# JzHuai0108/sim3opt

Hardware: AMD Instinct MI355X
Metric: LM iterations/s (higher is better)
Workload: dtype f64

## Files before the change

sim3opt_amd/csrc/amg_kernels.hpp:

```cpp
#pragma once

__global__ __launch_bounds__(WG) void k_amg_adjoint(int nb, const int32_t* __restrict__ row2v,
                                                    const Sim3* __restrict__ states,
                                                    double* __restrict__ P) {
  for (int i = blockIdx.x * WG + threadIdx.x; i < nb; i += gridDim.x * WG) {
  const Sim3 S = load_sim3(states + row2v[i]);
  double R[9];
  sim3::R_from_quat(S.q, R);
  double A[49];
#pragma unroll
  for (int k = 0; k < 49; ++k) A[k] = 0.0;
  const double t0 = S.t[0], t1 = S.t[1], t2 = S.t[2];
#pragma unroll
  for (int c = 0; c < 3; ++c) {
    const double v0 = R[c], v1 = R[3 + c], v2 = R[6 + c];
    A[0 + 7 * c] = v0;
    A[1 + 7 * c] = v1;
    A[2 + 7 * c] = v2;
    A[3 + 7 * c] = t1 * v2 - t2 * v1;
    A[4 + 7 * c] = t2 * v0 - t0 * v2;
    A[5 + 7 * c] = t0 * v1 - t1 * v0;
    A[3 + 7 * (3 + c)] = S.s * v0;
    A[4 + 7 * (3 + c)] = S.s * v1;
    A[5 + 7 * (3 + c)] = S.s * v2;
// ... 214 lines not shown
  const int sub = lane / 7, rr = lane % 7, base = lane - rr;
  for (int row0 = row_lo + (blockIdx.x * 4 + wave) * 9; row0 < row_hi; row0 += gridDim.x * 36) {
    const bool act = lane < 63 && row0 + sub < row_hi;
    const int row = act ? (list ? list[row0 + sub] : row0 + sub) : 0;
    const double xc = act ? x_c[(size_t)7 * agg[row] + rr] : 0.0;
    double add = xc;
    if (HASP) {
      add = 0.0;
#pragma unroll
      for (int m = 0; m < 7; ++m) {
        const double xm = __shfl(xc, base + m);
        if (act) add += P[(size_t)49 * row + rr + 7 * m] * xm;
      }
    }
    if (act) x_out[(size_t)7 * row + rr] = x_in[(size_t)7 * row + rr] + scale * add;
  }
}

constexpr int AMG_DENSE_MAX_N = 7 * AMG_MAX_COARSEST;
__global__ __launch_bounds__(WG) void k_amg_dense_fill(int nb, const int32_t* __restrict__ rowptr,
                                                       const int32_t* __restrict__ colidx,
                                                       const double* __restrict__ vals,
                                                       double* __restrict__ A,
                                                       const double* __restrict__ diag64 = nullptr) {
  const int n = 7 * nb;
  const int nnz = 49 * rowptr[nb];
  for (int t = blockIdx.x * WG + threadIdx.x; t < nnz; t += gridDim.x * WG) {
    const int k = t / 49, e = t % 49;
    int lo = 0, hi = nb;
    while (hi - lo > 1) {
      const int mid = (lo + hi) >> 1;
      if (rowptr[mid] <= k) lo = mid; else hi = mid;
    }
    const double v = diag64 && k == rowptr[lo] ? diag64[(size_t)49 * lo + e] : vals[(size_t)49 * k + e];
    A[(size_t)(7 * lo + e % 7) * n + 7 * colidx[k] + e / 7] = v;
  }
}


template <int NP>
__device__ inline bool gj_invert_rows(double (&prow)[NP], int lane) {
  bool spd = true;
#pragma unroll
  for (int k = 0; k < NP; ++k) {
    double pk[NP];
#pragma unroll
    for (int c = 0; c < NP; ++c) pk[c] = __shfl(prow[c], k);
// ... 47 lines not shown
#pragma unroll
    for (int c = 0; c < H; ++c) prow[c] = src[(size_t)rr * ld + H * h + c];
    spd = gj_invert_halfrows<NP>(prow, lane);
    if (r < NP) {
#pragma unroll
      for (int c = 0; c < H; ++c) Pout[r * NP + H * h + c] = prow[c];
    }
  } else {
    double prow[NP];
    const int rr = lane < NP ? lane : 0;
#pragma unroll
    for (int c = 0; c < NP; ++c) prow[c] = src[(size_t)rr * ld + c];
    spd = gj_invert_rows<NP>(prow, lane);
    if (lane < NP) {
#pragma unroll
      for (int c = 0; c < NP; ++c) Pout[lane * NP + c] = prow[c];
    }
  }
  if (!spd && lane == 0) sc->fail = 1;
}

template <int PB>
__global__ __launch_bounds__(64) void k_amg_dense_gj_first(int n, const double* __restrict__ A,
                                                           double* __restrict__ Pout, DevScalars* sc) {
  gj_invert_block<PB>(A, n, Pout, threadIdx.x, sc);
}

template <int PB>
__global__ __launch_bounds__(WG) __attribute__((amdgpu_waves_per_eu(2))) void k_amg_dense_gj_step(int n, int k0, const double* __restrict__ A,
                                                          double* __restrict__ B,
                                                          const double* __restrict__ Pin,
                                                          double* __restrict__ Pout, int pbn,
                                                          DevScalars* sc) {
  __shared__ double P[PB][PB + 1];
  __shared__ double ak[PB][64];
  __shared__ double rowk[PB][64];
  __shared__ double colk[64][PB + 1];
  const int tid = threadIdx.x;
  const bool ahead = blockIdx.y == 0;
  if (ahead && (blockIdx.x != 0 || pbn == 0)) return;
  const int ext = ahead ? pbn : 64;
  const int i0 = ahead ? k0 + PB : (int)(blockIdx.y - 1) * 64, j0 = ahead ? k0 + PB : (int)blockIdx.x * 64;
  const int ty = tid >> 4, tx = tid & 15;
  double v[4][4];
  if (ahead) {
#pragma unroll
    for (int e = 0; e < 4; ++e) {
      const int t = tid + WG * e;
      v[0][e] = t < ext * ext ? A[(size_t)(i0 + t / ext) * n + j0 + t % ext] : 0.0;
    }
  } else {
#pragma unroll
    for (int a = 0; a < 4; ++a)
#pragma unroll
      for (int b = 0; b < 4; ++b) {
        const int i = i0 + ty + 16 * a, j = j0 + tx + 16 * b;
        v[a][b] = i < n && j < n ? A[(size_t)i * n + j] : 0.0;
// ... 101 lines not shown
```

sim3opt_amd/csrc/batch_kernels.hpp:

```cpp
#pragma once

template <int K>
__global__ __launch_bounds__(WG) void k_final_sum2_k(const double* __restrict__ pa, const double* __restrict__ pb,
                                                     int n, int pstride, DevScalars* __restrict__ sc) {
  __shared__ double sh[4];
#pragma unroll
  for (int s = 0; s < K; ++s) {
    const double a = sum_partials(pa + (size_t)s * pstride, n, sh);
    const double b = sum_partials(pb + (size_t)s * pstride, n, sh);
    if (threadIdx.x == 0) {
      sc[s].tmp_pq = a;
      sc[s].tmp_rz = b;
    }
  }
}

template <int K>
__global__ __launch_bounds__(WG) void k_pcg_init_k(int r0, int r1, const double* __restrict__ b,
                                                   const double* __restrict__ Minv, double* __restrict__ x,
                                                   double* __restrict__ r, double* __restrict__ z,
                                                   double* __restrict__ p, double* __restrict__ sv,
                                                   BatchStrides bs) {
  const int lane = threadIdx.x & 63;
  const int wave = threadIdx.x >> 6;
  const int sub = lane / 7, rr = lane % 7, base = lane - rr;
  for (int row0 = r0 + (blockIdx.x * 4 + wave) * 9; row0 < r1; row0 += gridDim.x * 36) {
    const int row = row0 + sub;
    const bool act = lane < 63 && row < r1;
    const size_t j = (size_t)7 * row + rr;
    const double rv = act ? b[j] : 0.0;
#pragma unroll
    for (int s = 0; s < K; ++s) {
      const size_t o = (size_t)s * bs.vec;
      if (act) {
        x[o + j] = 0.0;
        r[o + j] = rv;
// ... 260 lines not shown
```

sim3opt_amd/csrc/engine_amg.hip:

```cpp
#include "engine_impl.hpp"

namespace sim3opt {

#include "spmv_kernel.hpp"
#include "amg_kernels.hpp"

int Engine::amg_init(const Structure& s, bool automatic, std::string& err) {
  (void)err;
  amg_omega = std::max(0.1, std::min(0.95, opt.amg_omega));
  amg_additive = opt.amg_additive != 0;
  {
    const bool partitioned = part_world() >= 2;
    int last = 0;
    for (int l = 1; l <= AMG_MAX_LEVELS; ++l) {
      const int o = l <= 4 ? opt.amg_cycle[l - 1] : 0;
      if (o >= 1 && o <= 3) last = o;
      amg_visits[l] = last > 0 ? last : (partitioned ? (l <= 1 ? 1 : 2) : (l <= 1 ? 2 : 3));
    }
    amg_visits[0] = 1;
  }
  amg_fp32 = opt.amg_fp32 != 0;
  adaptive_prec = opt.adaptive_prec != 0 && automatic;
  amg_pivot = opt.amg_pivot >= 28 ? 28 : 14;
  for (int l = 0; l <= AMG_MAX_LEVELS; ++l)
// ... 158 lines not shown
  }
  if (amg_fp32)
    for (int l = nl - 1; l < nl; ++l) {
      const size_t cnt = (size_t)49 * (size_t)amg[l].nnzb;
      hipLaunchKernelGGL(k_to_f32, dim3(grid_for((int64_t)(cnt / 4), WG)), dim3(WG), 0, stream, cnt,
                         (const double*)amg[l].vals, amg[l].vals32);
    }
  HIPCHK(hipGetLastError());
  amg_stale = false;
  return SIM3OPT_OK;
}

void Engine::amg_prepare(double lambda) {
  const int nl = (int)amg.size();
  for (int l = 0; l < nl; ++l) {
    const AmgLevel& L = amg[l];
    const int lo = L.lo, hi = L.hi;
    jacobi(lo, hi, L.rowptr, L.vals, lambda, L.Minv, l == 0 && amg_additive ? 1.0 : amg_omega, L.diagH, L.W,
           l > 0 ? L.vals32 : (float*)nullptr);
  }
  dense_inverse(nullptr, d_Ainv, d_sc);
}

void Engine::dense_inverse(const double* diag64, double* Aout, DevScalars* sc) {
  const int nl = (int)amg.size();
  const AmgLevel& Lc = amg[nl - 1];
  const int nd = 7 * Lc.nb;
  auto pivot_rows = [&](int k0) { return nd - k0 >= amg_pivot ? amg_pivot : (nd - k0 >= 14 ? 14 : 7); };
  int nsteps = 0;
  for (int k0 = 0; k0 < nd; k0 += pivot_rows(k0)) ++nsteps;
  double *src = nsteps % 2 ? d_Ainv2 : Aout, *dst = nsteps % 2 ? Aout : d_Ainv2;
  (void)hipMemsetAsync(src, 0, sizeof(double) * (size_t)nd * nd, stream);
  hipLaunchKernelGGL(k_amg_dense_fill, dim3(grid_for(49 * Lc.nnzb, WG)), dim3(WG), 0, stream, Lc.nb,
                     Lc.rowptr, Lc.colidx, Lc.vals, src, diag64);
  double *pin = d_piv, *pout = d_piv + 28 * 28;
  switch (pivot_rows(0)) {
    case 28: hipLaunchKernelGGL((k_amg_dense_gj_first<28>), dim3(1), dim3(64), 0, stream, nd, (const double*)src, pin, sc); break;
    case 14: hipLaunchKernelGGL((k_amg_dense_gj_first<14>), dim3(1), dim3(64), 0, stream, nd, (const double*)src, pin, sc); break;
    default: hipLaunchKernelGGL((k_amg_dense_gj_first<7>), dim3(1), dim3(64), 0, stream, nd, (const double*)src, pin, sc);
  }
  const dim3 gt((nd + 63) / 64, (nd + 63) / 64 + 1);
  for (int k0 = 0; k0 < nd;) {
    const int pb = pivot_rows(k0), pbn = k0 + pb < nd ? pivot_rows(k0 + pb) : 0;
    if (pb == 28)
      hipLaunchKernelGGL((k_amg_dense_gj_step<28>), gt, dim3(WG), 0, stream, nd, k0, (const double*)src,
                         dst, (const double*)pin, pout, pbn, sc);
    else if (pb == 14)
      hipLaunchKernelGGL((k_amg_dense_gj_step<14>), gt, dim3(WG), 0, stream, nd, k0, (const double*)src,
                         dst, (const double*)pin, pout, pbn, sc);
    else
      hipLaunchKernelGGL((k_amg_dense_gj_step<7>), gt, dim3(WG), 0, stream, nd, k0, (const double*)src,
                         dst, (const double*)pin, pout, pbn, sc);
    k0 += pb;
    std::swap(src, dst);
    std::swap(pin, pout);
  }
}

void Engine::spmv_mode(const AmgLevel& L, int mode, int level, const double* v, double* out,
               const double* rvec, const double* xc) {
  double* const rz_part = level == 0 && mode == 2 && !amg_additive ? d_part_b : nullptr;
#define AMG_SPMV(NTV, MODEV)                                                                     \
hipLaunchKernelGGL((k_spmv_span<8, NTV, MODEV>), dim3(L.span_grid), dim3(WG), 0, stream, L.nb,  \
                   L.wrow, L.rowptr, L.colidx, L.vals, v, out, 0.0, rz_part, rvec,              \
                   const_cast<double*>(xc), level == 0 ? d_sc : (DevScalars*)nullptr, L.Minv, 1,   \
                   (const int32_t*)L.agg, amg_over, BatchStrides{0, 0, 0, 0, 0}, (const float*)nullptr)
#define AMG_SPMV32(NTV, MODEV)                                                                    \
hipLaunchKernelGGL((k_spmv_span<(NTV) ? SIM3OPT_F32_CH : SIM3OPT_COARSE_CH, NTV, MODEV, float>), dim3(L.span_grid), dim3(WG), 0, stream,  \
                   L.nb, L.wrow, L.rowptr, L.colidx, (const float*)L.vals32, v, out, 0.0,         \
                   rz_part, rvec, const_cast<double*>(xc),                                        \
                   level == 0 ? d_sc : (DevScalars*)nullptr, L.Minv, 1, (const int32_t*)L.agg, amg_over, BatchStrides{0, 0, 0, 0, 0}, (const float*)nullptr)
  if (amg_fp32) {
    if (level == 0) { if (mode == 1) AMG_SPMV32(true, 1); else AMG_SPMV32(true, 2); }
    else { if (mode == 1) AMG_SPMV32(false, 1); else if (mode == 3) AMG_SPMV32(false, 3); else AMG_SPMV32(false, 2); }
  } else {
// ... 135 lines not shown
```

sim3opt_amd/csrc/engine_batch.hip:

```cpp
#include "engine_impl.hpp"

namespace sim3opt {

#include "spmv_kernel.hpp"
#include "batch_kernels.hpp"

static inline int64_t pad64(int64_t n) { return (n + 63) / 64 * 64; }

#define BATCH_DISPATCH(NS, ...) \
  do {                          \
    if ((NS) == 1) { constexpr int KS = 1; __VA_ARGS__; } \
    else if ((NS) == 2) { constexpr int KS = 2; __VA_ARGS__; } \
    else if ((NS) == 3) { constexpr int KS = 3; __VA_ARGS__; } \
    else { constexpr int KS = 4; __VA_ARGS__; } \
  } while (0)

int Engine::batch_alloc(std::string& err) {
  if (batch_ready) return SIM3OPT_OK;
  const int nl = (int)amg.size();
  auto alloc = [&](double*& p, size_t count) -> int {
    HIPCHK(dev_malloc((void**)&p, sizeof(double) * std::max<size_t>(count, 1)));
    batch_owned.push_back(p);
    HIPCHK(hipMemsetAsync(p, 0, sizeof(double) * std::max<size_t>(count, 1), stream));
    return SIM3OPT_OK;
// ... 8 lines not shown
  blv.assign(nl, BatchLevel());
  for (int l = 0; l < nl; ++l) {
    BatchLevel& B = blv[l];
    const AmgLevel& L = amg[l];
    B.vs = l == 0 ? b_vs : pad64(7 * (int64_t)L.nb);
    B.ms = (int64_t)49 * L.nb;
    int rc = alloc(B.Minv, (size_t)KB * B.ms);
    if (rc) return rc;
    if (l == 0) {
      B.r = b_r; B.x = b_z; B.t = b_az;
    } else {
      if ((rc = alloc(B.r, (size_t)KB * B.vs))) return rc;
      if ((rc = alloc(B.x, (size_t)KB * B.vs))) return rc;
      if ((rc = alloc(B.t, (size_t)KB * B.vs))) return rc;
      HIPCHK(dev_malloc((void**)&B.diag32, sizeof(float) * (size_t)KB * B.ms));
      batch_owned.push_back(B.diag32);
      HIPCHK(hipMemsetAsync(B.diag32, 0, sizeof(float) * (size_t)KB * B.ms, stream));
    }
  }
  const size_t nc = (size_t)7 * amg[nl - 1].nb;
  b_as = (int64_t)(nc * nc);
  int rc = alloc(b_Ainv, (size_t)KB * b_as);
  if (rc) return rc;
  if ((rc = alloc(b_diag64, (size_t)KB * 49 * amg[nl - 1].nb))) return rc;
  if ((rc = alloc(b_part_a, (size_t)KB * SPAN_GRID_MAX))) return rc;
  if ((rc = alloc(b_part_b, (size_t)KB * SPAN_GRID_MAX))) return rc;
  HIPCHK(dev_malloc((void**)&d_bsc, sizeof(DevScalars) * KB));
  batch_owned.push_back(d_bsc);
  HIPCHK(hipMemsetAsync(d_bsc, 0, sizeof(DevScalars) * KB, stream));
  HIPCHK(host_malloc((void**)&h_bsc, sizeof(DevScalars) * KB));
  batch_ready = true;
  return SIM3OPT_OK;
}

void Engine::batch_release() {
  for (void* p : batch_owned)
    if (p) dev_free(p);
  batch_owned.clear();
  if (h_bsc) host_free(h_bsc);
  h_bsc = nullptr;
  d_bsc = nullptr;
  blv.clear();
  batch_ready = false;
}

void Engine::b_spmv_mode(int level, int mode, const double* v, double* out, const double* rvec, const double* xc) {
// ... 72 lines not shown
  return other;
}

int Engine::pcg_batch(const double* lams, int nsys, int32_t* iters, double* rel_res, bool* capped, bool* usable,
                      std::string& err) {
  *usable = false;
  int rc = batch_alloc(err);
  if (rc) return rc;
  if (amg_stale) {
    rc = amg_setup(err);
    if (rc) return rc;
  }
  const int nl = (int)amg.size();
  const int max_it = opt.pcg_max_iters > 0 ? opt.pcg_max_iters : (n <= 50000 ? std::max(100, 2 * n) : 1000);
  for (int s = 0; s < KB; ++s) {
    DevScalars& h = h_bsc[s];
    std::memset(&h, 0, sizeof(DevScalars));
    h.max_iter = max_it;
    h.tol2 = opt.pcg_rel_tol * opt.pcg_rel_tol;
    h.lambda = s < nsys ? lams[s] : lams[nsys - 1];
    h.done = s < nsys ? 0 : 1;
  }
  HIPCHK(hipMemcpyAsync(d_bsc, h_bsc, sizeof(DevScalars) * KB, hipMemcpyHostToDevice, stream));
  for (int s = 0; s < nsys; ++s) {
    for (int l = 0; l < nl; ++l) {
      const AmgLevel& L = amg[l];
      const BatchLevel& B = blv[l];
      jacobi(0, L.nb, L.rowptr, L.vals, lams[s], B.Minv + (size_t)s * B.ms, amg_omega, L.diagH, L.W, nullptr,
             d_bsc + s, l == nl - 1 ? b_diag64 + (size_t)s * 49 * L.nb : nullptr,
             l > 0 ? B.diag32 + (size_t)s * B.ms : nullptr);
    }
    dense_inverse(b_diag64 + (size_t)s * 49 * amg[nl - 1].nb, b_Ainv + (size_t)s * b_as, d_bsc + s);
  }
  const int gv = grid_for((nb + 8) / 9, 4);
  const int gs = span_grid;
  const BatchLevel& B0 = blv[0];
  BatchStrides bs0{b_vs, B0.ms, 0, 0, SPAN_GRID_MAX};
  b_nsys = nsys;
  BATCH_DISPATCH(nsys, hipLaunchKernelGGL((k_pcg_init_k<KS>), dim3(gv), dim3(WG), 0, stream, 0, nb, (const double*)d_b,
                     (const double*)B0.Minv, b_x, b_r, b_z, b_p, b_s, bs0));
  HIPCHK(hipGetLastError());
  HIPCHK(hipMemcpyAsync(h_bsc, d_bsc, sizeof(DevScalars) * KB, hipMemcpyDeviceToHost, stream));
  HIPCHK(hipStreamSynchronize(stream));
  for (int s = 0; s < nsys; ++s)
    if (h_bsc[s].fail) return SIM3OPT_OK;
  b_cycle(0, b_z, b_az);
  const int chunk = std::min(4, std::max(1, opt.pcg_check_every));
  int it = 0, par = 0;
  for (;;) {
    HIPCHK(hipMemcpyAsync(h_bsc, d_bsc, sizeof(DevScalars) * KB, hipMemcpyDeviceToHost, stream));
    HIPCHK(hipStreamSynchronize(stream));
    int live = 0;
    for (int s = 0; s < nsys; ++s)
      if (!(h_bsc[s].done || h_bsc[s].stop || h_bsc[s].fail)) live = s + 1;
    if (live == 0 || it >= max_it) break;
    b_nsys = live;
    const int todo = std::min(chunk, max_it - it);
    for (int c = 0; c < todo; ++c) {
      BATCH_DISPATCH(live, hipLaunchKernelGGL((k_spmv_span<8, true, 0, double, KS, false>), dim3(gs), dim3(WG), 0, stream,
                         nb, d_wrow, d_rowptr, d_colidx, (const double*)d_vals, (const double*)b_az, b_q, 0.0, b_part_a,
                         (const double*)nullptr, b_part_b, d_bsc, (const double*)nullptr, 1, (const int32_t*)nullptr, 1.0,
                         bs0, (const float*)nullptr));
      BATCH_DISPATCH(live, hipLaunchKernelGGL((k_final_sum2_k<KS>), dim3(1), dim3(WG), 0, stream, (const double*)b_part_a,
                         (const double*)b_part_b, gs, SPAN_GRID_MAX, d_bsc));
      BATCH_DISPATCH(live, hipLaunchKernelGGL((k_pcg_step_k<KS>), dim3(gv), dim3(WG), 0, stream, 0, nb, par, it,
                         (const double*)B0.Minv, (const double*)b_az, b_z, (const double*)b_q, b_p, b_s, b_x, b_r, d_bsc,
                         bs0));
      b_cycle(0, b_z, b_az);
      par ^= 1;
      ++it;
    }
    HIPCHK(hipGetLastError());
  }
  bool good = true;
  for (int s = 0; s < nsys; ++s) {
    if (h_bsc[s].fail) { good = false; continue; }
    norms2(b_r + (size_t)s * b_vs, d_b, b_part_a, b_part_b, &d_bsc[s].tmp_pq);
  }
  HIPCHK(hipGetLastError());
  HIPCHK(hipMemcpyAsync(h_bsc, d_bsc, sizeof(DevScalars) * KB, hipMemcpyDeviceToHost, stream));
  HIPCHK(hipStreamSynchronize(stream));
  int it_max = 0;
  for (int s = 0; s < nsys; ++s) {
    const DevScalars& h = h_bsc[s];
    const double true_rel = h.tmp_rz > 0 ? std::sqrt(h.tmp_pq / h.tmp_rz) : 0.0;
    if (h.fail || true_rel > 1e-3) good = false;
// ... 17 lines not shown
```

sim3opt_amd/csrc/engine_impl.hpp:

```cpp
#pragma once
#include <hip/hip_runtime.h>
#include <hip/hip_ext.h>

#include <algorithm>
#include <cfloat>
#include <chrono>
#include <cmath>
#include <cstdio>
#include <cstddef>
#include <cstdlib>
#include <cstring>

#include "amg.hpp"
#include "comm.hpp"
#include "devmem.hpp"
#include "direct.hpp"
#include "engine.hpp"

namespace sim3opt {

using sim3::Sim3;

#define HIPCHK(call)                                                        \
  do {                                                                      \
// ... 128 lines not shown
  bool amg_additive = false;
  bool amg_fp32 = true;
  double amg_over_l[AMG_MAX_LEVELS + 1];
  double amg_over = 1.0;
  bool amg_over_on = true;
  int amg_pivot = 14;
  bool adaptive_prec = true;
  double bj_gate = -1.0;
  int bj_budget = 48;
  int n_bj_solves = 0, n_bj_abandoned = 0;
  bool trace_stale = true;
  double mean_diag = 0.0;
  int amg_status = 0;
  std::string amg_err;
  struct BatchLevel {
    double *Minv = nullptr, *r = nullptr, *x = nullptr, *t = nullptr;
    float* diag32 = nullptr;
    int64_t vs = 0, ms = 0;
  };
  std::vector<BatchLevel> blv;
  std::vector<void*> batch_owned;
  double *b_x = nullptr, *b_r = nullptr, *b_z = nullptr, *b_p = nullptr, *b_q = nullptr, *b_s = nullptr, *b_az = nullptr;
  double *b_Ainv = nullptr, *b_diag64 = nullptr, *b_part_a = nullptr, *b_part_b = nullptr;
  int64_t b_vs = 0, b_as = 0;
  DevScalars *d_bsc = nullptr, *h_bsc = nullptr;
  bool batch_ready = false;
  int b_nsys = KB;
  int64_t b_slice_blocks = 100000;
  int batch_alloc(std::string& err);
  void batch_release();
  void b_spmv_mode(int level, int mode, const double* v, double* out, const double* rvec, const double* xc);
  void b_restrict(int l, const double* t);
  double* b_coarse(int l);
  double* b_cycle(int l, double* cur, double* other);
  int pcg_batch(const double* lams, int nsys, int32_t* iters, double* rel_res, bool* capped, bool* usable,
                std::string& err);
  int batch_capacity() const {
    if (!use_amg || use_direct || comm.active() || !amg_fp32 || amg_additive || opt.pcg_batch == 1) return 0;
    return opt.pcg_batch > 1 ? std::min(opt.pcg_batch, KB) : KB;
  }
  DirectPlan dplan;
  bool use_direct = false;
  LdlArgs ldl{};
  int ldl_wg_sub = LDL_WG_SUB;
  int fail_token = 1;
  std::vector<void*> direct_owned;
// ... 101 lines not shown
  template <typename T>
  int direct_up(const T*& dptr, const std::vector<T>& h, std::string& err) {
    T* p = nullptr;
    HIPCHK(dev_malloc((void**)&p, sizeof(T) * std::max<size_t>(h.size(), 1)));
    direct_owned.push_back(p);
    if (!h.empty()) HIPCHK(staged.put(p, h.data(), sizeof(T) * h.size(), stream));
    dptr = p;
    return SIM3OPT_OK;
  }
  int direct_alloc(double*& dptr, size_t count, std::string& err) {
    HIPCHK(dev_malloc((void**)&dptr, sizeof(double) * std::max<size_t>(count, 1)));
    direct_owned.push_back(dptr);
    HIPCHK(hipMemset(dptr, 0, sizeof(double) * std::max<size_t>(count, 1)));
    return SIM3OPT_OK;
  }

  int direct_init(const Structure& s, std::string& err);

  int direct_solve(double lambda, std::string& err);
  void direct_gather();
  void jacobi(int lo, int hi, const int32_t* rowptr, double* vals, double lambda, double* Minv, double omega,
              const double* diagH, const double* W, float* vals32, DevScalars* sc = nullptr,
              double* diag64_out = nullptr, float* diag32_out = nullptr);
  void norms2(const double* r, const double* b, double* part_a, double* part_b, double* out2);
  void dense_inverse(const double* diag64, double* Aout, DevScalars* sc);

  int exchange_rows(double* vec, std::string& err) { return exchange_level(0, vec, err); }

  int chi2(double* out, std::string& err, hipEvent_t before_fetch = nullptr, int scale_parts = 0);

  Sim3* d_ptab = nullptr;
  double ptab_delta = 0.0;
  sim3::Opts ptab_opts{0.0, -1, -1};

  int linearize(std::string& err);

  int spmv_chunk = 8, spmv_nt = 1;

  int spmv_grid() const { return span_grid; }

  void spmv_raw(double lambda, const double* v, double* q, const double* rvec, DevScalars* scp,
                hipEvent_t ev0 = nullptr, hipEvent_t ev1 = nullptr);

  int spmv_launch(double lambda, const double* z, const double* rv, std::string& err);

  int agree_on_fail(std::string& err);

  int pcg(double lambda, int32_t* iters, double* rel_res, bool* ok, std::string& err);
// ... 9 lines not shown
```

sim3opt_amd/csrc/engine_pcg.hip:

```cpp
#include "engine_impl.hpp"

namespace sim3opt {

#include "spmv_kernel.hpp"
#include "pcg_kernels.hpp"

void Engine::jacobi(int lo, int hi, const int32_t* rowptr, double* vals, double lambda, double* Minv, double omega,
                    const double* diagH, const double* W, float* vals32, DevScalars* sc, double* diag64_out,
                    float* diag32_out) {
  hipLaunchKernelGGL(k_jacobi, dim3(std::max(1, (hi - lo + WG - 1) / WG)), dim3(WG), 0, stream, lo, hi, rowptr, vals,
                     lambda, Minv, sc ? sc : d_sc, omega, diagH, W, vals32, diag64_out, diag32_out);
}

void Engine::norms2(const double* r, const double* b, double* part_a, double* part_b, double* out2) {
  const int gn = grid_for(7 * (int64_t)(r1 - r0), WG);
  hipLaunchKernelGGL(k_norms2, dim3(gn), dim3(WG), 0, stream, 7 * r0, 7 * r1, r, b, part_a, part_b);
  hipLaunchKernelGGL(k_final_sum2, dim3(1), dim3(WG), 0, stream, part_a, part_b, gn, out2);
}

int Engine::level_part_init(int l, int32_t nb_l, const int32_t* rowptr_l, const int32_t* colidx_l,
                            const std::vector<int32_t>& row_begin_l, std::string& err) {
  LevelPart& lp = parts[l];
  lp.row_begin = row_begin_l;
  lp.lo = row_begin_l[comm.rank];
  lp.hi = row_begin_l[comm.rank + 1];
  lp.offs.resize(comm.world + 1);
  lp.blk_offs.resize(comm.world + 1);
  for (int r = 0; r <= comm.world; ++r) {
    lp.offs[r] = 7 * (int64_t)row_begin_l[r];
    lp.blk_offs[r] = 49 * (int64_t)rowptr_l[row_begin_l[r]];
  }
  if (!opt.halo_exchange || !comm.can_exchange()) return SIM3OPT_OK;
  std::vector<int32_t> srows, sseg, rrows, rseg;
  if (comm.world <= 1) {
// ... 399 lines not shown
```

sim3opt_amd/csrc/pcg_kernels.hpp:

```cpp
#pragma once
__global__ __launch_bounds__(WG) void k_final_sum2(const double* __restrict__ pa,
                                                   const double* __restrict__ pb, int n,
                                                   double* __restrict__ out2) {
  __shared__ double sh[4];
  const double a = sum_partials(pa, n, sh);
  const double b = sum_partials(pb, n, sh);
  if (threadIdx.x == 0) {
    out2[0] = a;
    out2[1] = b;
  }
}

__global__ void k_fail_to_double(DevScalars* sc) { sc->tmp_pq = sc->fail ? 1.0 : 0.0; }
__global__ void k_double_to_fail(DevScalars* sc) { if (sc->tmp_pq > 0.0) sc->fail = 1; }

__global__ __launch_bounds__(WG) void k_jacobi(int r0, int r1, const int32_t* __restrict__ rowptr,
                                               double* __restrict__ vals, double lambda,
                                               double* __restrict__ Minv, DevScalars* sc,
                                               double omega, const double* __restrict__ diagH,
                                               const double* __restrict__ W,
                                               float* __restrict__ vals32 = nullptr,
                                               double* __restrict__ diag64_out = nullptr,
                                               float* __restrict__ diag32_out = nullptr) {
  const int row = r0 + blockIdx.x * WG + threadIdx.x;
  if (row >= r1) return;
  double a[7][7];
  double* blk = vals + (size_t)49 * rowptr[row];
  const int64_t kd = rowptr[row];
  const double* src = diagH ? diagH + (size_t)49 * row : blk;
#pragma unroll
  for (int c = 0; c < 7; ++c)
#pragma unroll
    for (int r = 0; r < 7; ++r) a[r][c] = src[7 * c + r];
  if (W) {
    const double* w = W + (size_t)49 * row;
#pragma unroll
    for (int c = 0; c < 7; ++c)
#pragma unroll
      for (int r = 0; r < 7; ++r) {
        a[r][c] += lambda * w[7 * c + r];
        if (diag64_out || diag32_out) {
          if (diag64_out) diag64_out[(size_t)49 * row + 7 * c + r] = a[r][c];
          if (diag32_out) diag32_out[(size_t)49 * row + 7 * c + r] = (float)a[r][c];
        } else {
          blk[7 * c + r] = a[r][c];
          if (vals32) vals32[f32_pair_index(kd, 7 * c + r)] = (float)a[r][c];
        }
      }
  } else {
#pragma unroll
    for (int i = 0; i < 7; ++i) a[i][i] += lambda;
  }
  bool spd = true;
#pragma unroll
  for (int k = 0; k < 7; ++k) {
    if (!(a[k][k] > 0.0)) spd = false;
    const double d = 1.0 / a[k][k];
#pragma unroll
    for (int j = 0; j < 7; ++j)
      if (j != k) a[k][j] *= d;
#pragma unroll
    for (int i = 0; i < 7; ++i)
      if (i != k) {
        const double f = a[i][k];
#pragma unroll
        for (int j = 0; j < 7; ++j)
          if (j != k) a[i][j] -= f * a[k][j];
        a[i][k] = -f * d;
      }
    a[k][k] = d;
  }
  if (!spd) sc->fail = 1;
  double* dst = Minv + (size_t)49 * row;
#pragma unroll
  for (int r = 0; r < 7; ++r)
#pragma unroll
    for (int c = 0; c < 7; ++c) dst[7 * r + c] = omega * a[r][c];
}

__global__ __launch_bounds__(WG) void k_pcg_init(int r0, int r1, const double* __restrict__ b,
                                                 const double* __restrict__ Minv,
                                                 double* __restrict__ x, double* __restrict__ r,
                                                 double* __restrict__ z, double* __restrict__ p,
                                                 double* __restrict__ sv) {
  const int lane = threadIdx.x & 63;
  const int wave = threadIdx.x >> 6;
  const int sub = lane / 7, rr = lane % 7, base = lane - rr;
  for (int row0 = r0 + (blockIdx.x * 4 + wave) * 9; row0 < r1; row0 += gridDim.x * 36) {
    const int row = row0 + sub;
    const bool act = lane < 63 && row < r1;
    const size_t j = (size_t)7 * row + rr;
    const double rv = act ? b[j] : 0.0;
    if (act) {
      x[j] = 0.0;
      r[j] = rv;
      p[j] = 0.0;
      sv[j] = 0.0;
    }
    if (Minv) {
      double zv = 0.0;
// ... 275 lines not shown
```

sim3opt_amd/csrc/spmv_kernel.hpp:

```cpp
#pragma once
#ifndef SIM3OPT_SPMV_FASTPATH
#define SIM3OPT_SPMV_FASTPATH 1
#endif
constexpr bool FASTPATH = SIM3OPT_SPMV_FASTPATH != 0;

struct BatchStrides {
  int64_t vec;
  int64_t minv;
  int64_t xc;
  int64_t diag;
  int part;
};

#ifndef SIM3OPT_BATCH_WAVES
#define SIM3OPT_BATCH_WAVES 0
#endif
template <int CH, bool NT, int MODE, typename VT = double, int K = 1, bool DIAGK = false>
__global__ __launch_bounds__(WG)
#if SIM3OPT_BATCH_WAVES > 0
__attribute__((amdgpu_waves_per_eu(SIM3OPT_BATCH_WAVES, SIM3OPT_BATCH_WAVES)))
#endif
void k_spmv_span(int nb, const int32_t* __restrict__ wrow,
                                                  const int32_t* __restrict__ rowptr,
                                                  const int32_t* __restrict__ colidx,
                                                  const VT* __restrict__ vals,
                                                  const double* __restrict__ p,
                                                  double* __restrict__ q, double lambda,
                                                  double* __restrict__ partials,
                                                  const double* __restrict__ rvec,
                                                  double* __restrict__ partials_r,
                                                  DevScalars* __restrict__ sc,
                                                  const double* __restrict__ Minv, int lam_sc,
                                                  const int32_t* __restrict__ agg,
                                                  double xc_scale, BatchStrides bs,
                                                  const float* __restrict__ diagk) {
  __shared__ double sh[K][4];
  __shared__ double sh2[K][4];
  __shared__ int sh_cnt;
#ifndef SIM3OPT_X_LDS
#define SIM3OPT_X_LDS 1
#endif
  constexpr bool XLDS = SIM3OPT_X_LDS != 0 && !(sizeof(VT) == 8 && K > 1);
  constexpr int NGX = (CH + 7) / 8;
  __shared__ double xl[XLDS ? 4 : 1][XLDS ? K : 1][XLDS ? NGX : 1][64];
  double (*xw)[NGX][64] = xl[XLDS ? (threadIdx.x >> 6) : 0];
#ifndef SIM3OPT_ROWEND_LDS
#define SIM3OPT_ROWEND_LDS 1
#endif
  constexpr bool RLDS = XLDS && SIM3OPT_ROWEND_LDS != 0;
  __shared__ __attribute__((aligned(16))) double rl[XLDS ? 4 : 1][64];
  double* const rw = rl[XLDS ? (threadIdx.x >> 6) : 0];
  if (MODE == 2 || MODE == 0) {
    if (threadIdx.x == 0) sh_cnt = 0;
    __syncthreads();
  }
  if (gridDim.y > 1) {
    const size_t s0 = (size_t)blockIdx.y * K;
    p += s0 * bs.vec;
    q += s0 * bs.vec;
    if (rvec) rvec += s0 * bs.vec;
    if (Minv) Minv += s0 * bs.minv;
    if (MODE == 3) partials_r += s0 * bs.xc;
    if (DIAGK) diagk += s0 * bs.diag;
    if (partials) partials += s0 * bs.part;
    if (sc) sc += s0;
  }
  double lam[K];
#pragma unroll
  for (int s = 0; s < K; ++s) lam[s] = lambda;
  if (sc) {
    bool all_done = true;
#pragma unroll
    for (int s = 0; s < K; ++s) all_done = all_done && sc[s].done;
    if (all_done) return;
    if (lam_sc) {
#pragma unroll
      for (int s = 0; s < K; ++s) lam[s] = sc[s].lambda;
    }
// ... 15 lines not shown
  double pq[K], pr[K];
  double pi_n[K], rv_n[K], mv[K], acc[K];
#pragma unroll
  for (int s = 0; s < K; ++s) pq[s] = pr[s] = pi_n[s] = rv_n[s] = mv[s] = acc[s] = 0.0;
  int kfirst = 0;
  auto xget = [&](const double (*xg)[NG], int s, int u, int src) -> double {
    if (XLDS) return xw[s][u / 8][src];
    return __shfl(xg[s][u / 8], src);
  };
  auto xstage = [&](const double (*xg)[NG]) {
    if (XLDS) {
      wave_lds_sync();
#pragma unroll
      for (int s = 0; s < K; ++s)
#pragma unroll
        for (int g = 0; g < NG; ++g) xw[s][g][threadIdx.x & 63] = xg[s][g];
      wave_lds_sync();
    }
  };
  auto row_begin = [&](int row, int u, const double (*xg)[NG]) {
#pragma unroll
    for (int s = 0; s < K; ++s) {
      pi_n[s] = xget(xg, s, u, 7 * (u % 8) + r);
      if (rvec) rv_n[s] = rvec[(size_t)s * bs.vec + (size_t)7 * row + r];
      if (MODE >= 2) mv[s] = Minv[(size_t)s * bs.minv + (size_t)49 * row + l49];
      if (DIAGK)
        acc[s] = (double)diagk[(size_t)s * bs.diag + (size_t)49 * row + l49] * xget(xg, s, u, 7 * (u % 8) + c49);
      else
        acc[s] = 0.0;
    }
  };
  typedef double d2_t __attribute__((ext_vector_type(2)));
  auto colsum = [&](double v) -> double {
    if (RLDS) {
      wave_lds_sync();
      rw[8 * r + c49] = v;
      wave_lds_sync();
      const d2_t* pp = reinterpret_cast<const d2_t*>(rw + 8 * (lane < 7 ? lane : 0));
      const d2_t a = pp[0], b = pp[1], c = pp[2];
      const double e = rw[8 * (lane < 7 ? lane : 0) + 6];
      return (((((a.x + a.y) + b.x) + b.y) + c.x) + c.y) + e;
    }
    double y = v;
#pragma unroll
    for (int cc = 1; cc < 7; ++cc) y += __shfl(v, r + 7 * cc);
    return y;
  };
  auto row_end = [&](int row) {
#pragma unroll
    for (int s = 0; s < K; ++s) {
      double y = colsum(acc[s]);
      const double pi = pi_n[s];
      y += lam[s] * pi;
      double* qs = q + (size_t)s * bs.vec;
      if (MODE == 0) {
        if (lane < 7) {
          qs[(size_t)7 * row + lane] = y;
          pq[s] += pi * y;
          if (rvec) pr[s] += rv_n[s] * pi;
        }
      } else {
        const double d = rv_n[s] - y;
        if (MODE == 1) {
          if (lane < 7) qs[(size_t)7 * row + lane] = d;
        } else {
          double dc;
          if (RLDS) {
            if (lane < 7) rw[56 + lane] = d;
            wave_lds_sync();
            dc = rw[56 + c49];
          } else {
            dc = __shfl(d, c49);
          }
          const double pr_ = mv[s] * dc;
          const double o = colsum(pr_);
          if (lane < 7) {
            const double zo = pi + o;
            qs[(size_t)7 * row + lane] = zo;
            if (MODE == 2 && partials) pr[s] += rv_n[s] * zo;
          }
        }
      }
// ... 115 lines not shown
  if (MODE == 2 && partials) {
    double t[K];
#pragma unroll
    for (int s = 0; s < K; ++s) t[s] = wave_sum(pr[s]);
    if (lane == 0) {
#pragma unroll
      for (int s = 0; s < K; ++s) sh[s][threadIdx.x >> 6] = t[s];
      __threadfence_block();
      if (atomicAdd(&sh_cnt, 1) == 3) {
        __threadfence_block();
#pragma unroll
        for (int s = 0; s < K; ++s)
          partials[(size_t)s * bs.part + blockIdx.x] = (sh[s][0] + sh[s][1]) + (sh[s][2] + sh[s][3]);
      }
    }
    return;
  }
  if (MODE != 0) return;
  {
    double sa[K], sb[K];
#pragma unroll
    for (int s = 0; s < K; ++s) {
      sa[s] = wave_sum(pq[s]);
      sb[s] = rvec ? wave_sum(pr[s]) : 0.0;
    }
    if (lane == 0) {
#pragma unroll
      for (int s = 0; s < K; ++s) {
        sh[s][threadIdx.x >> 6] = sa[s];
        sh2[s][threadIdx.x >> 6] = sb[s];
      }
      __threadfence_block();
      if (atomicAdd(&sh_cnt, 1) == 3) {
        __threadfence_block();
#pragma unroll
        for (int s = 0; s < K; ++s) {
          if (partials) partials[(size_t)s * bs.part + blockIdx.x] = (sh[s][0] + sh[s][1]) + (sh[s][2] + sh[s][3]);
          if (rvec) partials_r[(size_t)s * bs.part + blockIdx.x] = (sh2[s][0] + sh2[s][1]) + (sh2[s][2] + sh2[s][3]);
        }
      }
    }
  }
}
```

Measured before the change: 47.55.

## Batch per-system Jacobi and dense inverse setup across grid dimension

Replaces the per-system host loop of jacobi and dense_inverse launches with single launches that index systems through an extra grid dimension. This adds dedicated scratch buffers for the alternate matrix and the pivots. The final partial-sum kernel now runs one block per system instead of looping in a single block. It also enables LDS staging of x for f64 multi-system SpMV and makes the rvec check a compile-time condition. The aim is to cut launch count and serialisation, at the cost of extra memory and a changed LDS and register profile in the batched SpMV.

```diff
diff --git a/sim3opt_amd/csrc/amg_kernels.hpp b/sim3opt_amd/csrc/amg_kernels.hpp
--- a/sim3opt_amd/csrc/amg_kernels.hpp
+++ b/sim3opt_amd/csrc/amg_kernels.hpp
@@ -260,7 +260,12 @@
                                                        const int32_t* __restrict__ colidx,
                                                        const double* __restrict__ vals,
                                                        double* __restrict__ A,
-                                                       const double* __restrict__ diag64 = nullptr) {
+                                                       const double* __restrict__ diag64 = nullptr,
+                                                       int64_t as = 0) {
+  if (gridDim.y > 1) {
+    A += blockIdx.y * as;
+    diag64 += (size_t)blockIdx.y * 49 * nb;
+  }
   const int n = 7 * nb;
   const int nnz = 49 * rowptr[nb];
   for (int t = blockIdx.x * WG + threadIdx.x; t < nnz; t += gridDim.x * WG) {
@@ -354,7 +359,13 @@
 
 template <int PB>
 __global__ __launch_bounds__(64) void k_amg_dense_gj_first(int n, const double* __restrict__ A,
-                                                           double* __restrict__ Pout, DevScalars* sc) {
+                                                           double* __restrict__ Pout, DevScalars* sc,
+                                                           int64_t as = 0, int64_t ps = 0) {
+  if (gridDim.y > 1) {
+    A += blockIdx.y * as;
+    Pout += blockIdx.y * ps;
+    sc += blockIdx.y;
+  }
   gj_invert_block<PB>(A, n, Pout, threadIdx.x, sc);
 }
 
@@ -363,8 +374,15 @@
                                                           double* __restrict__ B,
                                                           const double* __restrict__ Pin,
                                                           double* __restrict__ Pout, int pbn,
-                                                          DevScalars* sc) {
+                                                          DevScalars* sc, int64_t as = 0, int64_t ps = 0) {
   __shared__ double P[PB][PB + 1];
+  if (gridDim.z > 1) {
+    A += blockIdx.z * as;
+    B += blockIdx.z * as;
+    Pin += blockIdx.z * ps;
+    Pout += blockIdx.z * ps;
+    sc += blockIdx.z;
+  }
   __shared__ double ak[PB][64];
   __shared__ double rowk[PB][64];
   __shared__ double colk[64][PB + 1];
diff --git a/sim3opt_amd/csrc/batch_kernels.hpp b/sim3opt_amd/csrc/batch_kernels.hpp
--- a/sim3opt_amd/csrc/batch_kernels.hpp
+++ b/sim3opt_amd/csrc/batch_kernels.hpp
@@ -4,14 +4,13 @@
 __global__ __launch_bounds__(WG) void k_final_sum2_k(const double* __restrict__ pa, const double* __restrict__ pb,
                                                      int n, int pstride, DevScalars* __restrict__ sc) {
   __shared__ double sh[4];
-#pragma unroll
-  for (int s = 0; s < K; ++s) {
-    const double a = sum_partials(pa + (size_t)s * pstride, n, sh);
-    const double b = sum_partials(pb + (size_t)s * pstride, n, sh);
-    if (threadIdx.x == 0) {
-      sc[s].tmp_pq = a;
-      sc[s].tmp_rz = b;
-    }
+  const int s = blockIdx.x;
+  if (s >= K) return;
+  const double a = sum_partials(pa + (size_t)s * pstride, n, sh);
+  const double b = sum_partials(pb + (size_t)s * pstride, n, sh);
+  if (threadIdx.x == 0) {
+    sc[s].tmp_pq = a;
+    sc[s].tmp_rz = b;
   }
 }
 
diff --git a/sim3opt_amd/csrc/engine_amg.hip b/sim3opt_amd/csrc/engine_amg.hip
--- a/sim3opt_amd/csrc/engine_amg.hip
+++ b/sim3opt_amd/csrc/engine_amg.hip
@@ -204,35 +204,40 @@
   dense_inverse(nullptr, d_Ainv, d_sc);
 }
 
-void Engine::dense_inverse(const double* diag64, double* Aout, DevScalars* sc) {
+void Engine::dense_inverse(const double* diag64, double* Aout, DevScalars* sc, int nsys, double* Aalt,
+                           double* piv) {
   const int nl = (int)amg.size();
   const AmgLevel& Lc = amg[nl - 1];
   const int nd = 7 * Lc.nb;
+  if (!Aalt) Aalt = d_Ainv2;
+  if (!piv) piv = d_piv;
+  const int64_t as = (int64_t)nd * nd, ps = 2 * 28 * 28;
   auto pivot_rows = [&](int k0) { return nd - k0 >= amg_pivot ? amg_pivot : (nd - k0 >= 14 ? 14 : 7); };
   int nsteps = 0;
   for (int k0 = 0; k0 < nd; k0 += pivot_rows(k0)) ++nsteps;
-  double *src = nsteps % 2 ? d_Ainv2 : Aout, *dst = nsteps % 2 ? Aout : d_Ainv2;
-  (void)hipMemsetAsync(src, 0, sizeof(double) * (size_t)nd * nd, stream);
-  hipLaunchKernelGGL(k_amg_dense_fill, dim3(grid_for(49 * Lc.nnzb, WG)), dim3(WG), 0, stream, Lc.nb,
-                     Lc.rowptr, Lc.colidx, Lc.vals, src, diag64);
-  double *pin = d_piv, *pout = d_piv + 28 * 28;
+  double *src = nsteps % 2 ? Aalt : Aout, *dst = nsteps % 2 ? Aout : Aalt;
+  (void)hipMemsetAsync(src, 0, sizeof(double) * (size_t)nsys * as, stream);
+  hipLaunchKernelGGL(k_amg_dense_fill, dim3(grid_for(49 * Lc.nnzb, WG), nsys), dim3(WG), 0, stream, Lc.nb,
+                     Lc.rowptr, Lc.colidx, Lc.vals, src, diag64, as);
+  double *pin = piv, *pout = piv + 28 * 28;
+  const dim3 g1(1, nsys);
   switch (pivot_rows(0)) {
-    case 28: hipLaunchKernelGGL((k_amg_dense_gj_first<28>), dim3(1), dim3(64), 0, stream, nd, (const double*)src, pin, sc); break;
-    case 14: hipLaunchKernelGGL((k_amg_dense_gj_first<14>), dim3(1), dim3(64), 0, stream, nd, (const double*)src, pin, sc); break;
-    default: hipLaunchKernelGGL((k_amg_dense_gj_first<7>), dim3(1), dim3(64), 0, stream, nd, (const double*)src, pin, sc);
-  }
-  const dim3 gt((nd + 63) / 64, (nd + 63) / 64 + 1);
+    case 28: hipLaunchKernelGGL((k_amg_dense_gj_first<28>), g1, dim3(64), 0, stream, nd, (const double*)src, pin, sc, as, ps); break;
+    case 14: hipLaunchKernelGGL((k_amg_dense_gj_first<14>), g1, dim3(64), 0, stream, nd, (const double*)src, pin, sc, as, ps); break;
+    default: hipLaunchKernelGGL((k_amg_dense_gj_first<7>), g1, dim3(64), 0, stream, nd, (const double*)src, pin, sc, as, ps);
+  }
+  const dim3 gt((nd + 63) / 64, (nd + 63) / 64 + 1, nsys);
   for (int k0 = 0; k0 < nd;) {
     const int pb = pivot_rows(k0), pbn = k0 + pb < nd ? pivot_rows(k0 + pb) : 0;
     if (pb == 28)
       hipLaunchKernelGGL((k_amg_dense_gj_step<28>), gt, dim3(WG), 0, stream, nd, k0, (const double*)src,
-                         dst, (const double*)pin, pout, pbn, sc);
+                         dst, (const double*)pin, pout, pbn, sc, as, ps);
     else if (pb == 14)
       hipLaunchKernelGGL((k_amg_dense_gj_step<14>), gt, dim3(WG), 0, stream, nd, k0, (const double*)src,
-                         dst, (const double*)pin, pout, pbn, sc);
+                         dst, (const double*)pin, pout, pbn, sc, as, ps);
     else
       hipLaunchKernelGGL((k_amg_dense_gj_step<7>), gt, dim3(WG), 0, stream, nd, k0, (const double*)src,
-                         dst, (const double*)pin, pout, pbn, sc);
+                         dst, (const double*)pin, pout, pbn, sc, as, ps);
     k0 += pb;
     std::swap(src, dst);
     std::swap(pin, pout);
diff --git a/sim3opt_amd/csrc/engine_batch.hip b/sim3opt_amd/csrc/engine_batch.hip
--- a/sim3opt_amd/csrc/engine_batch.hip
+++ b/sim3opt_amd/csrc/engine_batch.hip
@@ -54,6 +54,8 @@
   b_as = (int64_t)(nc * nc);
   int rc = alloc(b_Ainv, (size_t)KB * b_as);
   if (rc) return rc;
+  if ((rc = alloc(b_Ainv2, (size_t)KB * b_as))) return rc;
+  if ((rc = alloc(b_piv, (size_t)KB * 2 * 28 * 28))) return rc;
   if ((rc = alloc(b_diag64, (size_t)KB * 49 * amg[nl - 1].nb))) return rc;
   if ((rc = alloc(b_part_a, (size_t)KB * SPAN_GRID_MAX))) return rc;
   if ((rc = alloc(b_part_b, (size_t)KB * SPAN_GRID_MAX))) return rc;
@@ -172,16 +174,13 @@
     h.done = s < nsys ? 0 : 1;
   }
   HIPCHK(hipMemcpyAsync(d_bsc, h_bsc, sizeof(DevScalars) * KB, hipMemcpyHostToDevice, stream));
-  for (int s = 0; s < nsys; ++s) {
-    for (int l = 0; l < nl; ++l) {
-      const AmgLevel& L = amg[l];
-      const BatchLevel& B = blv[l];
-      jacobi(0, L.nb, L.rowptr, L.vals, lams[s], B.Minv + (size_t)s * B.ms, amg_omega, L.diagH, L.W, nullptr,
-             d_bsc + s, l == nl - 1 ? b_diag64 + (size_t)s * 49 * L.nb : nullptr,
-             l > 0 ? B.diag32 + (size_t)s * B.ms : nullptr);
-    }
-    dense_inverse(b_diag64 + (size_t)s * 49 * amg[nl - 1].nb, b_Ainv + (size_t)s * b_as, d_bsc + s);
-  }
+  for (int l = 0; l < nl; ++l) {
+    const AmgLevel& L = amg[l];
+    const BatchLevel& B = blv[l];
+    jacobi_k(L.nb, L.rowptr, L.vals, lams, nsys, B.Minv, B.ms, amg_omega, L.diagH, L.W, d_bsc,
+             l == nl - 1 ? b_diag64 : nullptr, l > 0 ? B.diag32 : nullptr);
+  }
+  dense_inverse(b_diag64, b_Ainv, d_bsc, nsys, b_Ainv2, b_piv);
   const int gv = grid_for((nb + 8) / 9, 4);
   const int gs = span_grid;
   const BatchLevel& B0 = blv[0];
@@ -211,7 +210,7 @@
                          nb, d_wrow, d_rowptr, d_colidx, (const double*)d_vals, (const double*)b_az, b_q, 0.0, b_part_a,
                          (const double*)nullptr, b_part_b, d_bsc, (const double*)nullptr, 1, (const int32_t*)nullptr, 1.0,
                          bs0, (const float*)nullptr));
-      BATCH_DISPATCH(live, hipLaunchKernelGGL((k_final_sum2_k<KS>), dim3(1), dim3(WG), 0, stream, (const double*)b_part_a,
+      BATCH_DISPATCH(live, hipLaunchKernelGGL((k_final_sum2_k<KS>), dim3(KS), dim3(WG), 0, stream, (const double*)b_part_a,
                          (const double*)b_part_b, gs, SPAN_GRID_MAX, d_bsc));
       BATCH_DISPATCH(live, hipLaunchKernelGGL((k_pcg_step_k<KS>), dim3(gv), dim3(WG), 0, stream, 0, nb, par, it,
                          (const double*)B0.Minv, (const double*)b_az, b_z, (const double*)b_q, b_p, b_s, b_x, b_r, d_bsc,
diff --git a/sim3opt_amd/csrc/engine_impl.hpp b/sim3opt_amd/csrc/engine_impl.hpp
--- a/sim3opt_amd/csrc/engine_impl.hpp
+++ b/sim3opt_amd/csrc/engine_impl.hpp
@@ -174,6 +174,7 @@
   std::vector<void*> batch_owned;
   double *b_x = nullptr, *b_r = nullptr, *b_z = nullptr, *b_p = nullptr, *b_q = nullptr, *b_s = nullptr, *b_az = nullptr;
   double *b_Ainv = nullptr, *b_diag64 = nullptr, *b_part_a = nullptr, *b_part_b = nullptr;
+  double *b_Ainv2 = nullptr, *b_piv = nullptr;
   int64_t b_vs = 0, b_as = 0;
   DevScalars *d_bsc = nullptr, *h_bsc = nullptr;
   bool batch_ready = false;
@@ -321,8 +322,12 @@
   void jacobi(int lo, int hi, const int32_t* rowptr, double* vals, double lambda, double* Minv, double omega,
               const double* diagH, const double* W, float* vals32, DevScalars* sc = nullptr,
               double* diag64_out = nullptr, float* diag32_out = nullptr);
+  void jacobi_k(int nb_l, const int32_t* rowptr, double* vals, const double* lams, int nsys, double* Minv, int64_t ms,
+                double omega, const double* diagH, const double* W, DevScalars* sc, double* diag64_out,
+                float* diag32_out);
   void norms2(const double* r, const double* b, double* part_a, double* part_b, double* out2);
-  void dense_inverse(const double* diag64, double* Aout, DevScalars* sc);
+  void dense_inverse(const double* diag64, double* Aout, DevScalars* sc, int nsys = 1, double* Aalt = nullptr,
+                     double* piv = nullptr);
 
   int exchange_rows(double* vec, std::string& err) { return exchange_level(0, vec, err); }
 
diff --git a/sim3opt_amd/csrc/engine_pcg.hip b/sim3opt_amd/csrc/engine_pcg.hip
--- a/sim3opt_amd/csrc/engine_pcg.hip
+++ b/sim3opt_amd/csrc/engine_pcg.hip
@@ -10,6 +10,16 @@
                     float* diag32_out) {
   hipLaunchKernelGGL(k_jacobi, dim3(std::max(1, (hi - lo + WG - 1) / WG)), dim3(WG), 0, stream, lo, hi, rowptr, vals,
                      lambda, Minv, sc ? sc : d_sc, omega, diagH, W, vals32, diag64_out, diag32_out);
+}
+
+void Engine::jacobi_k(int nb_l, const int32_t* rowptr, double* vals, const double* lams, int nsys, double* Minv,
+                      int64_t ms, double omega, const double* diagH, const double* W, DevScalars* sc,
+                      double* diag64_out, float* diag32_out) {
+  static_assert(KB <= (int)(sizeof(BatchLams::v) / sizeof(double)), "one damping per system of a batch");
+  BatchLams bl{};
+  for (int s = 0; s < nsys; ++s) bl.v[s] = lams[s];
+  hipLaunchKernelGGL(k_jacobi_k, dim3(std::max(1, (nb_l + WG - 1) / WG), nsys), dim3(WG), 0, stream, 0, nb_l, rowptr,
+                     vals, bl, Minv, ms, sc, omega, diagH, W, diag64_out, diag32_out, ms);
 }
 
 void Engine::norms2(const double* r, const double* b, double* part_a, double* part_b, double* out2) {
diff --git a/sim3opt_amd/csrc/pcg_kernels.hpp b/sim3opt_amd/csrc/pcg_kernels.hpp
--- a/sim3opt_amd/csrc/pcg_kernels.hpp
+++ b/sim3opt_amd/csrc/pcg_kernels.hpp
@@ -14,6 +14,65 @@
 __global__ void k_fail_to_double(DevScalars* sc) { sc->tmp_pq = sc->fail ? 1.0 : 0.0; }
 __global__ void k_double_to_fail(DevScalars* sc) { if (sc->tmp_pq > 0.0) sc->fail = 1; }
 
+__device__ __forceinline__ void jacobi_row(int row, const int32_t* __restrict__ rowptr, double* __restrict__ vals,
+                                           double lambda, double* __restrict__ Minv, DevScalars* sc, double omega,
+                                           const double* __restrict__ diagH, const double* __restrict__ W,
+                                           float* __restrict__ vals32, double* __restrict__ diag64_out,
+                                           float* __restrict__ diag32_out) {
+  double a[7][7];
+  double* blk = vals + (size_t)49 * rowptr[row];
+  const int64_t kd = rowptr[row];
+  const double* src = diagH ? diagH + (size_t)49 * row : blk;
+#pragma unroll
+  for (int c = 0; c < 7; ++c)
+#pragma unroll
+    for (int r = 0; r < 7; ++r) a[r][c] = src[7 * c + r];
+  if (W) {
+    const double* w = W + (size_t)49 * row;
+#pragma unroll
+    for (int c = 0; c < 7; ++c)
+#pragma unroll
+      for (int r = 0; r < 7; ++r) {
+        a[r][c] += lambda * w[7 * c + r];
+        if (diag64_out || diag32_out) {
+          if (diag64_out) diag64_out[(size_t)49 * row + 7 * c + r] = a[r][c];
+          if (diag32_out) diag32_out[(size_t)49 * row + 7 * c + r] = (float)a[r][c];
+        } else {
+          blk[7 * c + r] = a[r][c];
+          if (vals32) vals32[f32_pair_index(kd, 7 * c + r)] = (float)a[r][c];
+        }
+      }
+  } else {
+#pragma unroll
+    for (int i = 0; i < 7; ++i) a[i][i] += lambda;
+  }
+  bool spd = true;
+#pragma unroll
+  for (int k = 0; k < 7; ++k) {
+    if (!(a[k][k] > 0.0)) spd = false;
+    const double d = 1.0 / a[k][k];
+#pragma unroll
+    for (int j = 0; j < 7; ++j)
+      if (j != k) a[k][j] *= d;
+#pragma unroll
+    for (int i = 0; i < 7; ++i)
+      if (i != k) {
+        const double f = a[i][k];
+#pragma unroll
+        for (int j = 0; j < 7; ++j)
+          if (j != k) a[i][j] -= f * a[k][j];
+        a[i][k] = -f * d;
+      }
+    a[k][k] = d;
+  }
+  if (!spd) sc->fail = 1;
+  double* dst = Minv + (size_t)49 * row;
+#pragma unroll
+  for (int r = 0; r < 7; ++r)
+#pragma unroll
+    for (int c = 0; c < 7; ++c) dst[7 * r + c] = omega * a[r][c];
+}
+
 __global__ __launch_bounds__(WG) void k_jacobi(int r0, int r1, const int32_t* __restrict__ rowptr,
                                                double* __restrict__ vals, double lambda,
                                                double* __restrict__ Minv, DevScalars* sc,
@@ -24,58 +83,24 @@
                                                float* __restrict__ diag32_out = nullptr) {
   const int row = r0 + blockIdx.x * WG + threadIdx.x;
   if (row >= r1) return;
-  double a[7][7];
-  double* blk = vals + (size_t)49 * rowptr[row];
-  const int64_t kd = rowptr[row];
-  const double* src = diagH ? diagH + (size_t)49 * row : blk;
-#pragma unroll
-  for (int c = 0; c < 7; ++c)
-#pragma unroll
-    for (int r = 0; r < 7; ++r) a[r][c] = src[7 * c + r];
-  if (W) {
-    const double* w = W + (size_t)49 * row;
-#pragma unroll
-    for (int c = 0; c < 7; ++c)
-#pragma unroll
-      for (int r = 0; r < 7; ++r) {
-        a[r][c] += lambda * w[7 * c + r];
-        if (diag64_out || diag32_out) {
-          if (diag64_out) diag64_out[(size_t)49 * row + 7 * c + r] = a[r][c];
-          if (diag32_out) diag32_out[(size_t)49 * row + 7 * c + r] = (float)a[r][c];
-        } else {
-          blk[7 * c + r] = a[r][c];
-          if (vals32) vals32[f32_pair_index(kd, 7 * c + r)] = (float)a[r][c];
-        }
-      }
-  } else {
-#pragma unroll
-    for (int i = 0; i < 7; ++i) a[i][i] += lambda;
-  }
-  bool spd = true;
-#pragma unroll
-  for (int k = 0; k < 7; ++k) {
-    if (!(a[k][k] > 0.0)) spd = false;
-    const double d = 1.0 / a[k][k];
-#pragma unroll
-    for (int j = 0; j < 7; ++j)
-      if (j != k) a[k][j] *= d;
-#pragma unroll
-    for (int i = 0; i < 7; ++i)
-      if (i != k) {
-        const double f = a[i][k];
-#pragma unroll
-        for (int j = 0; j < 7; ++j)
-          if (j != k) a[i][j] -= f * a[k][j];
-        a[i][k] = -f * d;
-      }
-    a[k][k] = d;
-  }
-  if (!spd) sc->fail = 1;
-  double* dst = Minv + (size_t)49 * row;
-#pragma unroll
-  for (int r = 0; r < 7; ++r)
-#pragma unroll
-    for (int c = 0; c < 7; ++c) dst[7 * r + c] = omega * a[r][c];
+  jacobi_row(row, rowptr, vals, lambda, Minv, sc, omega, diagH, W, vals32, diag64_out, diag32_out);
+}
+
+struct BatchLams {
+  double v[4];
+};
+
+__global__ __launch_bounds__(WG) void k_jacobi_k(int r0, int r1, const int32_t* __restrict__ rowptr,
+                                                 double* __restrict__ vals, BatchLams lam, double* __restrict__ Minv,
+                                                 int64_t ms, DevScalars* sc, double omega,
+                                                 const double* __restrict__ diagH, const double* __restrict__ W,
+                                                 double* __restrict__ diag64_out, float* __restrict__ diag32_out,
+                                                 int64_t ds) {
+  const int row = r0 + blockIdx.x * WG + threadIdx.x;
+  if (row >= r1) return;
+  const int s = blockIdx.y;
+  jacobi_row(row, rowptr, vals, lam.v[s], Minv + s * ms, sc + s, omega, diagH, W, nullptr,
+             diag64_out ? diag64_out + s * ds : nullptr, diag32_out ? diag32_out + s * ds : nullptr);
 }
 
 __global__ __launch_bounds__(WG) void k_pcg_init(int r0, int r1, const double* __restrict__ b,
diff --git a/sim3opt_amd/csrc/spmv_kernel.hpp b/sim3opt_amd/csrc/spmv_kernel.hpp
--- a/sim3opt_amd/csrc/spmv_kernel.hpp
+++ b/sim3opt_amd/csrc/spmv_kernel.hpp
@@ -40,7 +40,10 @@
 #ifndef SIM3OPT_X_LDS
 #define SIM3OPT_X_LDS 1
 #endif
-  constexpr bool XLDS = SIM3OPT_X_LDS != 0 && !(sizeof(VT) == 8 && K > 1);
+#ifndef SIM3OPT_X_LDS_F64K
+#define SIM3OPT_X_LDS_F64K 1
+#endif
+  constexpr bool XLDS = SIM3OPT_X_LDS != 0 && (SIM3OPT_X_LDS_F64K != 0 || !(sizeof(VT) == 8 && K > 1));
   constexpr int NGX = (CH + 7) / 8;
   __shared__ double xl[XLDS ? 4 : 1][XLDS ? K : 1][XLDS ? NGX : 1][64];
   double (*xw)[NGX][64] = xl[XLDS ? (threadIdx.x >> 6) : 0];
@@ -54,6 +57,7 @@
     if (threadIdx.x == 0) sh_cnt = 0;
     __syncthreads();
   }
+  auto has_rvec = [&]() -> bool { return K > 1 ? MODE != 0 : rvec != nullptr; };
   if (gridDim.y > 1) {
     const size_t s0 = (size_t)blockIdx.y * K;
     p += s0 * bs.vec;
@@ -115,7 +119,7 @@
 #pragma unroll
     for (int s = 0; s < K; ++s) {
       pi_n[s] = xget(xg, s, u, 7 * (u % 8) + r);
-      if (rvec) rv_n[s] = rvec[(size_t)s * bs.vec + (size_t)7 * row + r];
+      if (has_rvec()) rv_n[s] = rvec[(size_t)s * bs.vec + (size_t)7 * row + r];
       if (MODE >= 2) mv[s] = Minv[(size_t)s * bs.minv + (size_t)49 * row + l49];
       if (DIAGK)
         acc[s] = (double)diagk[(size_t)s * bs.diag + (size_t)49 * row + l49] * xget(xg, s, u, 7 * (u % 8) + c49);
@@ -150,7 +154,7 @@
         if (lane < 7) {
           qs[(size_t)7 * row + lane] = y;
           pq[s] += pi * y;
-          if (rvec) pr[s] += rv_n[s] * pi;
+          if (has_rvec()) pr[s] += rv_n[s] * pi;
         }
       } else {
         const double d = rv_n[s] - y;
@@ -312,7 +316,7 @@
 #pragma unroll
     for (int s = 0; s < K; ++s) {
       sa[s] = wave_sum(pq[s]);
-      sb[s] = rvec ? wave_sum(pr[s]) : 0.0;
+      sb[s] = has_rvec() ? wave_sum(pr[s]) : 0.0;
     }
     if (lane == 0) {
 #pragma unroll
@@ -326,7 +330,7 @@
 #pragma unroll
         for (int s = 0; s < K; ++s) {
           if (partials) partials[(size_t)s * bs.part + blockIdx.x] = (sh[s][0] + sh[s][1]) + (sh[s][2] + sh[s][3]);
-          if (rvec) partials_r[(size_t)s * bs.part + blockIdx.x] = (sh2[s][0] + sh2[s][1]) + (sh2[s][2] + sh2[s][3]);
+          if (has_rvec()) partials_r[(size_t)s * bs.part + blockIdx.x] = (sh2[s][0] + sh2[s][1]) + (sh2[s][2] + sh2[s][3]);
         }
       }
     }
```

Measured after the change: 48.93 (median of 6 runs). 1.03x the previous value.
